# brandonckelly/carma_pack

Measured on AMD Instinct MI355X. Metric: Kalman log-lik evals/sec, CARMA(5,3) n=270, higher is better.
Workload: dtype f64

## Files before the change

### carma_pack_amd/csrc/carma_pipew.h

```cpp
#pragma once
#include <hip/hip_runtime.h>

#include "carma_core.h"
#include "grp_device.h"
#include "carma_pipe3l.h"
#include "carma_win_asm.h"

namespace carma {

#if defined(CARMA_STAMPS)
#define PIPEW_MARK(i) do { if (mk) { __builtin_amdgcn_sched_barrier(0); mk[i] = clock64(); __builtin_amdgcn_sched_barrier(0); } } while (0)
#else
#define PIPEW_MARK(i) do { } while (0)
#endif

template <int P>
struct PipeWGeom {
    static constexpr int ND = 16 - P;
    static constexpr int NB = 2;
    static constexpr int ENT = P + 1;
    static constexpr int RING_OFF = 0;
    static constexpr int ROT_OFF = NB * ENT * 64;
    static constexpr int HDR_OFF = ROT_OFF + NB * P * 4;
    static constexpr int CONST_OFF = HDR_OFF + NB;
    static constexpr int OUT_OFF = CONST_OFF + 64;
    static constexpr int TAB_OFF = OUT_OFF + 4;
    static constexpr int MRG_OFF = TAB_OFF + MATH_TAB_N / 2;
    static constexpr int MRG_STRIDE = P + 1 + ((P + 1) & 1);
    static constexpr int MRG_X = 0;
    static constexpr int MRG_COL = MRG_X + P * MRG_STRIDE;
    static constexpr int MRG_L = MRG_COL + MRG_STRIDE;
    static constexpr int MRG_T = MRG_L + P * MRG_STRIDE;
    static constexpr int MRG_DOUBLES = MRG_T + P * MRG_STRIDE;
    static constexpr int TH_OFF = MRG_OFF + (2 * MRG_DOUBLES + 1) / 2;
    static constexpr int SCH_OFF = TH_OFF + 128;
    static constexpr int ENTRIES = SCH_OFF + NB * 4 * 2;
    static constexpr int SER_OFF = ENTRIES;
    static __host__ __device__ size_t bytes_with_series(int n) { return BYTES + (size_t)(n + (n & 1)) * 24; }
    static constexpr int NPROD = 3;
    static constexpr size_t BYTES = (size_t)ENTRIES * sizeof(double2);
    static constexpr double LIM_RE = Pipe3LGeom<P>::LIM_RE, LIM_IM = Pipe3LGeom<P>::LIM_IM;
};

CARMA_DEV double exp_step_tab_exact(double a, double dt, const double* tab)
{
    const double x = a * dt;
    const double n1 = rint(x * INV_LN2_32);
    double r = fma3(-n1, LN2_32_HI, x);
    r = fma3(-n1, LN2_32_LO, r);
    r += fma3(a, dt, -x);
    const int i1 = (int)fmin(fmax(n1, -70400.0), 70400.0);
    const double e0 = tab[i1 & 31];
    double pe = 1.0 / 720.0;
    pe = fma3(pe, r, 1.0 / 120.0);
    pe = fma3(pe, r, 1.0 / 24.0);
    pe = fma3(pe, r, 1.0 / 6.0);
    pe = fma3(pe, r, 0.5);
    pe = fma3(pe, r, 1.0);
    return ldexp(fma3(e0, pe * r, e0), i1 >> 5);
}

template <int P, bool TS = false, bool SLDS = false, bool HANDOVER = false, bool FOLD = false, class Tail>
__device__ __forceinline__ void pipew_produce(const Grp<16>& g, int pw, const double* __restrict__ theta,
                                              const double4* __restrict__ series, int n_all, double2* __restrict__ ring, Tail&& tail,
                                              long long* mk = nullptr, const double* __restrict__ lds_t = nullptr,
                                              const double2* __restrict__ lds_yz = nullptr)
{
    using Geo = PipeWGeom<P>;
    constexpr int ND = Geo::ND, NB = Geo::NB, ENT = Geo::ENT;
    if (CARMA_PRIO_P != 0) __builtin_amdgcn_s_setprio(CARMA_PRIO_P);
    static_assert(!FOLD || ((P & 1) && P >= 3 && TS && SLDS && HANDOVER), "the folded form: odd orders of the two-sided kernel with the hand-over");
    constexpr int NPAIR = FOLD ? P / 2 : (P + 1) / 2, PPL = 16 / NPAIR;
    constexpr int NPROD = FOLD ? 2 : Geo::NPROD;
    constexpr int PWD = TS ? 2 : 0;
    constexpr int PWH = FOLD ? 2 : 0;
    constexpr int NIT = (ND + 1 + NPROD * PPL - 1) / (NPROD * PPL);
    const double* tab = reinterpret_cast<const double*>(ring + Geo::TAB_OFF);
    const int lane = g.lane64, l = lane & 15, rowb = lane & ~15, q = lane >> 4;
    const int sub = l / NPAIR, jr = 2 * (l - sub * NPAIR);
    const bool worker = sub < PPL, two = FOLD ? true : jr + 1 < P;
    const bool fold = FOLD && jr == P - 3;
    const bool bwd = TS && (q & 1);
    const int nfwd = (n_all + 1) / 2;
    const int n = TS ? (bwd ? n_all - nfwd : nfwd) : n_all;
    auto recat = [=](int j) {
        const int jj = j < n ? j : n - 1;
        double4 r = series[bwd ? n_all - 1 - jj : jj];
        if (bwd) r.w = -r.w;
        return r;
    };
    int jw = 0;
    double4 rw0, rw1, rw2, rw3;
    if constexpr (!SLDS) {
        rw0 = recat(l);
        rw1 = recat(16 + l);
        rw2 = recat(32 + l);
        rw3 = recat(48 + l);
    }
    auto sidx = [=](int j) {
        const int jj = j < n ? j : n - 1;
        return bwd ? n_all - 1 - jj : jj;
    };
    const double tsgn = bwd ? -1.0 : 1.0;
    double t_first = 0.0, t_meet = 0.0;
    if constexpr (!SLDS) {
        t_first = recat(0).w;
        t_meet = TS ? (bwd ? -series[nfwd - 1].w : series[nfwd - 1].w) : 0.0;
    }
    Cx w = own_ar_root<P>(theta, jr);
    Cx w1 = two ? own_ar_root<P>(theta, jr + 1) : w;
    if (bwd) {
        w.im = -w.im;
        w1.im = -w1.im;
    }
    Cx ws = {0.0, 0.0};
    if constexpr (FOLD) {
        ws = own_ar_root<P>(theta, P - 1);
        if (bwd) ws.im = -ws.im;
    }
    int esig = 0;
    {
        const double sg = fabs(theta[0]);
        (void)frexp(sg, &esig);
        if (!(sg > 0.0 && sg < 1.0 / 0.0)) esig = 0;
    }
    const double mu = theta[2], scale = theta[1];
    const bool realpair = two && w.im == 0.0;
    if (pw == PWH && l >= ND) {
#pragma unroll
        for (int b = 0; b < NB; b++) {
#pragma unroll
            for (int r = 0; r < P; r++) ring[Geo::RING_OFF + (b * ENT + r) * 64 + lane] = make_double2(r == l - ND ? 1.0 : 0.0, 0.0);
            ring[Geo::RING_OFF + (b * ENT + P) * 64 + lane] = make_double2(1.0, 0.0);
        }
    }
    double wl = fmax(fmax(fabs(w.re), fabs(w1.re)) * (1.0 / Geo::LIM_RE), fabs(w.im) * (1.0 / Geo::LIM_IM));
    wl = (wl < 1e12) ? wl : ((wl == wl && wl < 1.0 / 0.0) ? 1e12 : 0.0);
    if constexpr (FOLD) {
        double wls = fmax(fabs(ws.re) * (1.0 / Geo::LIM_RE), fabs(ws.im) * (1.0 / Geo::LIM_IM));
        wls = (wls < 1e12) ? wls : ((wls == wls && wls < 1.0 / 0.0) ? 1e12 : 0.0);
        wl = fmax(wl, wls);
    }
    wl = Grp<16>::max(wl);
    int wex;
    (void)frexp(wl, &wex);
    const double sc = wl > 0.0 ? ldexp(1.0, wex) : 0.0;
    const double halfw = sc > 0.0 ? 0.5 / sc : 0.0;
    const double rg0 = exp_neg(w.re * halfw), g0 = recip(rg0);
    double rg1 = rg0, g1 = g0;
    if (realpair) {
        rg1 = exp_neg(w1.re * halfw);
        g1 = recip(rg1);
    }
    double gS = 1.0;
    if constexpr (FOLD) gS = recip(exp_neg(ws.re * halfw));
    int j0 = 0;
    double base = t_first;
    constexpr bool SSCHED = TS && SLDS && HANDOVER;
    int len = 0, jc = 0;
    bool rot = false, last = false, fin = false;
    double dt_rot = 0.0, dta_keep = 0.0;
    double2 dslot = make_double2(1.0, 0.0);
    unsigned long long rbits = 0ull;
    double ecv[NIT], esv[NIT], e1v[NIT];
    double exv[NIT];
    auto sched = [&](bool finflag) __attribute__((always_inline)) {
        jc = j0;
        const int jl = j0 + l;
        double4 rec;
        if constexpr (SLDS) {
            const int si = sidx(jl);
            rec.x = rec.y = rec.z = 0.0;
            rec.w = tsgn * lds_t[si];
            if (pw == PWD) {
                const double2 yz = lds_yz[si];
                rec.y = yz.x;
                rec.z = yz.y;
            }
        } else {
            const int pos = jl - jw, src = rowb + (pos & 15);
            const bool hi = pos >= 16;
            const double w0 = __shfl(rw0.w, src, 64), w1_ = __shfl(rw1.w, src, 64);
            rec.x = rec.y = rec.z = 0.0;
            rec.w = hi ? w1_ : w0;
            if (pw == PWD) {
                const double y0 = __shfl(rw0.y, src, 64), y1 = __shfl(rw1.y, src, 64);
                const double z0 = __shfl(rw0.z, src, 64), z1 = __shfl(rw1.z, src, 64);
                rec.y = hi ? y1 : y0;
                rec.z = hi ? z1 : z0;
            }
        }
        const double tj = rec.w;
        const int left = n - j0;
        const int ncand = left < ND ? (left > 0 ? left : 0) : ND;
        const double t0 = finflag ? t_meet : Grp<16>::template bcast_c<0>(tj);
        const double t_lastc = SLDS ? tsgn * lds_t[sidx(j0 + (ncand > 0 ? ncand - 1 : 0))] : __shfl(tj, rowb + (ncand > 0 ? ncand - 1 : 0), 64);
        const double W = sc > 0.0 ? 1.0 / sc : 1.0 / 0.0;
        rot = finflag || (ncand > 0 && (t_lastc - base) > W);
        dt_rot = t0 - base;
        base = rot ? t0 : base;
        const double dta_l = tj - base;
        dta_keep = dta_l;
        const unsigned long long flb = __ballot(dta_l > W && l < ncand);
        const unsigned cut = (unsigned)(flb >> (16 * q)) & 0xffffu;
        len = cut ? __builtin_ctz(cut) : ncand;
        const bool row_done = j0 + len >= n;
        last = __ballot(!row_done) == 0ull;
        if (pw == PWD) dslot = l < len ? make_double2(rec.z * scale, rec.y - mu) : make_double2(1.0, 0.0);
        j0 += len;
        if (!SLDS && j0 - jw >= 16) {
            rw0 = rw1;
            rw1 = rw2;
            rw2 = rw3;
            jw += 16;
            rw3 = recat(jw + 48 + l);
        }
    };
    double2* schb = ring + Geo::SCH_OFF;
    auto sched_put = [&](int b) __attribute__((always_inline)) {
        if (l == 0) {
            const int bits = jc | (len << 16) | (rot ? 1 << 24 : 0) | (last ? 1 << 25 : 0);
            schb[(b * 4 + q) * 2] = make_double2(__hiloint2double(0, bits), base);
            schb[(b * 4 + q) * 2 + 1] = make_double2(dt_rot, 0.0);
        }
    };
    auto sched_get = [&](int b) __attribute__((always_inline)) {
        const double2 s0 = schb[(b * 4 + q) * 2], s1 = schb[(b * 4 + q) * 2 + 1];
        const int bits = __double2loint(s0.x);
        jc = bits & 0xffff;
        len = (bits >> 16) & 0xff;
        rot = ((bits >> 24) & 1) != 0;
        last = ((bits >> 25) & 1) != 0;
        base = s0.y;
        dt_rot = s1.x;
    };
    auto exps = [&]() __attribute__((always_inline)) {
        if (pw == PWH) rbits = __ballot(rot);
        if constexpr (FOLD) {
            if (pw >= NPROD) return;
        }
#pragma unroll
        for (int it = 0; it < NIT; it++) {
            const int slot = it * NPROD * PPL + pw * PPL + sub;
            const bool is_rot = slot == ND;
            double dts;
            if constexpr (SLDS) {
                dts = tsgn * lds_t[sidx(jc + (slot < ND ? slot : 0))] - base;
            } else {
                dts = __shfl(dta_keep, rowb + (slot < ND ? slot : 0), 64);
            }
            const double dt = is_rot ? dt_rot : dts;
            const bool live = worker && (is_rot ? rot : slot < len);
            double ec = 1.0, es = 0.0, e1 = 1.0;
            if (live) cexp_step_tab<true>(w.re, w.im, dt, &ec, &es, tab);
            e1 = ec;
            if (realpair && live) e1 = exp_neg_tab(w1.re * dt, tab);
            ecv[it] = ec;
            esv[it] = es;
            e1v[it] = e1;
            if constexpr (FOLD) exv[it] = (fold && live) ? exp_step_tab_exact(ws.re, dt, tab) : 1.0;
        }
    };
    PIPEW_MARK(1);
    __syncthreads();
    PIPEW_MARK(2);
    if constexpr (SLDS) {
        base = tsgn * lds_t[sidx(0)];
        t_meet = tsgn * lds_t[nfwd - 1];
    }
    double2 hc_own, hc_par, hc_s = make_double2(0.0, 0.0);
    {
        const double2* cst = ring + Geo::CONST_OFF + rowb;
        if constexpr (FOLD) {
            hc_s = cst[P - 1];
            const double ms = fabs(hc_s.x);
            int es_;
            (void)frexp(ms, &es_);
            if (!(ms > 0.0 && ms < 1.0 / 0.0)) es_ = 0;
            hc_s = make_double2(ldexp(hc_s.x, esig - es_), ldexp(hc_s.y, es_ - esig));
            if (bwd) hc_s = make_double2(hc_s.y, hc_s.x);
        }
        hc_own = cst[jr];
        hc_par = cst[jr + 1 < 16 ? jr + 1 : 15];
        const double m0 = fmax(fabs(hc_own.x), realpair ? 0.0 : fabs(hc_par.x)), m1 = realpair ? fabs(hc_par.x) : m0;
        int e0, e1x;
        (void)frexp(m0, &e0);
        (void)frexp(m1, &e1x);
        if (!(m0 > 0.0 && m0 < 1.0 / 0.0)) e0 = 0;
        if (!(m1 > 0.0 && m1 < 1.0 / 0.0)) e1x = 0;
        hc_own = make_double2(ldexp(hc_own.x, esig - e0), ldexp(hc_own.y, e0 - esig));
        hc_par = make_double2(ldexp(hc_par.x, esig - e1x), ldexp(hc_par.y, e1x - esig));
        if (bwd) {
            hc_own = make_double2(hc_own.y, hc_own.x);
            hc_par = make_double2(hc_par.y, hc_par.x);
        }
    }
#if defined(CARMA_WIN_STAMPS)
    unsigned long long ps_work = 0, ps_wait = 0, ps_t0 = 0, ps_t1 = 0;
    int ps_n = 0;
#define WIN_STAMP(v) asm volatile("s_memtime %0\n\ts_waitcnt lgkmcnt(0)" : "=s"(v)::"memory")
#endif
    for (int c = 0;; c++) {
        const int b = c % NB;
#if defined(CARMA_WIN_STAMPS)
        WIN_STAMP(ps_t0);
#endif
        if (!SSCHED || c == 0)
            sched(fin);
        else if (pw != PWD)
            sched_get(b);
        exps();
        if (pw == PWH && lane == 0)
            reinterpret_cast<unsigned long long*>(ring + Geo::HDR_OFF)[b] =
                ((rbits & 1ull) | ((rbits >> 15) & 2ull) | ((rbits >> 30) & 4ull) | ((rbits >> 45) & 8ull)) | ((TS ? fin : last) ? 256ull : 0ull);
        if (pw == PWD && l < ND) ring[Geo::RING_OFF + (b * ENT + P) * 64 + lane] = dslot;
        if (!FOLD || pw < NPROD) {
#pragma unroll
        for (int it = 0; it < NIT; it++) {
            const int slot = it * NPROD * PPL + pw * PPL + sub;
            const bool is_rot = slot == ND;
            const bool live = worker && (is_rot ? rot : slot < len);
            const double ec = ecv[it], es = esv[it], e1 = e1v[it];
            if (worker && slot < ND) {
                const double gc = ec * g0, gs = es * g0;
                const double inv = recip(fma(gc, gc, gs * gs));
                const double ht = fma(gc, hc_own.x, gs * hc_par.x);
                const double ct = fma(gc, hc_own.y, gs * hc_par.y) * inv;
                double2* dst = ring + Geo::RING_OFF + (b * ENT + jr) * 64 + rowb + slot;
                dst[0] = live ? make_double2(ht, ct) : make_double2(0.0, 0.0);
                if (two) {
                    const double gc1 = e1 * g1, gs1 = es * g1;
                    const double inv1 = realpair ? recip(gc1 * gc1) : inv;
                    const double hp = fma(gc1, hc_par.x, -gs1 * hc_own.x);
                    const double cp = fma(gc1, hc_par.y, -gs1 * hc_own.y) * inv1;
                    dst[64] = live ? make_double2(hp, cp) : make_double2(0.0, 0.0);
                }
                if constexpr (FOLD) {
                    if (fold) {
                        const double ex = exv[it], ez = ex * 0.0;
                        const double gcs = ex * gS, gss = ez * gS;
                        const double invs = recip(fma(gcs, gcs, gss * gss));
                        const double hts = fma(gcs, hc_s.x, gss * 0.0);
                        const double cts = fma(gcs, hc_s.y, gss * 0.0) * invs;
                        dst[128] = live ? make_double2(hts, cts) : make_double2(0.0, 0.0);
                    }
                }
            }
            if (worker && is_rot) {
                double2* dst = ring + Geo::ROT_OFF + (b * P + jr) * 4 + q;
                const double f0 = fin ? g0 : 1.0, f1 = fin ? g1 : 1.0;
                dst[0] = make_double2(ec * f0, es * f0);
                if (two) dst[4] = make_double2(e1 * f1, -es * f1);
                if constexpr (FOLD) {
                    if (fold) {
                        const double ex = exv[it], ez = ex * 0.0;
                        const double fS = fin ? gS : 1.0;
                        dst[8] = make_double2(ex * fS, ez * fS);
                    }
                }
            }
        }
        }
#if defined(CARMA_WIN_STAMPS)
        WIN_STAMP(ps_t1);
        ps_work += ps_t1 - ps_t0;
#endif
        const bool last_c = last, fin_c = fin;
        if (SSCHED && pw == PWD && !(TS ? fin_c : last_c)) {
            sched(last_c);
            sched_put((c + 1) % NB);
        }
        if (c < 3) PIPEW_MARK(3 + 2 * c - (c == 2));
        __syncthreads();
        if (c == 0) PIPEW_MARK(4);
#if defined(CARMA_WIN_STAMPS)
        WIN_STAMP(ps_t0);
        ps_wait += ps_t0 - ps_t1;
        ps_n++;
#endif
        if (TS ? fin_c : last_c) break;
        fin = last_c;
    }
#if defined(CARMA_WIN_STAMPS)
    if (blockIdx.x == 0 && lane == 0)
        printf("window pipeline, producer %d: %d chunks, per chunk %llu cycles of work, %llu at the barrier\n", pw, ps_n,
               ps_work / (unsigned long long)ps_n, ps_wait / (unsigned long long)ps_n);
#endif
    tail(pw);
    if (!TS) __syncthreads();
}

CARMA_DEV double rsqrt_pos(double d)
{
#ifdef __HIPCC__
    const double y0 = __builtin_amdgcn_rsq(d);
    const double e = fma(-d * y0, y0, 1.0);
    return fma(y0, fma(0.375 * e, e, 0.5 * e), y0);
#else
    return 1.0 / sqrt(d);
#endif
}
CARMA_DEV void merge_lds_sync()
{
#ifdef __HIPCC__
    __builtin_amdgcn_fence(__ATOMIC_RELEASE, "wavefront");
    __builtin_amdgcn_wave_barrier();
    __builtin_amdgcn_fence(__ATOMIC_ACQUIRE, "wavefront");
#endif
}
template <int P>
__device__ __forceinline__ void pipew_merge(int lane, const double (&kf)[P], double nu, double2* __restrict__ ring, LogLikAcc& acc,
                                            long long* mk = nullptr)
{
    using Geo = PipeWGeom<P>;
    constexpr int ND = Geo::ND, ST = Geo::MRG_STRIDE;
    const int l = lane & 15, q = lane >> 4;
    const bool bwd = (q & 1) != 0, virt = l >= ND;
    const int j = virt ? l - ND : 0;
    double* mrg = reinterpret_cast<double*>(ring + Geo::MRG_OFF) + (q >> 1) * Geo::MRG_DOUBLES;
    if (!bwd && virt) {
        double* dst = mrg + Geo::MRG_X + j * ST;
#pragma unroll
        for (int r = 0; r < P; r++) dst[r] = kf[r];
        dst[P] = nu;
    }
    merge_lds_sync();
    double S[P], av[P];
#pragma unroll
    for (int i = 0; i < P; i++) {
        S[i] = -mrg[Geo::MRG_X + (i >= j ? j * ST + i : i * ST + j)];
        av[i] = mrg[Geo::MRG_X + i * ST + P];
    }
    double aj = mrg[Geo::MRG_X + j * ST + P];
    int sj = 0;
    double dg = -mrg[Geo::MRG_X + j * ST + j];
    {
        int ex;
        (void)frexp(dg, &ex);
        if (dg > 0.0 && dg < 1.0 / 0.0) sj = -(ex >> 1);
    }
    dg = ldexp(dg, 2 * sj);
    double kfs[P];
    static_for<0, P>([&](auto ic) __attribute__((always_inline)) {
        constexpr int i = decltype(ic)::value;
        const int si = Grp<16>::template bcast_c<ND + i>(sj);
        S[i] = ldexp(S[i], si + sj);
        kfs[i] = ldexp(kf[i], -si - sj);
        av[i] = ldexp(av[i], si);
    });
    aj = ldexp(aj, sj);
    nu = ldexp(nu, -sj);
    PIPEW_MARK(8);
    double Lr[P];
#pragma unroll
    for (int i = 0; i < P; i++) Lr[i] = 0.0;
    bool done = !virt;
    bool exhausted = false;
    static_for<0, P>([&](auto mc) __attribute__((always_inline)) {
        constexpr int m = decltype(mc)::value;
        if (exhausted) return;
        const bool cand = !done && dg > 4e-15;
        unsigned key = cand ? (((unsigned)__double2hiint(dg) & ~0xFu) | (unsigned)(15 - l)) : 0u;
        const double r_own = cand ? rsqrt_pos(dg) : 0.0;
#ifdef __HIPCC__
        key = max(key, (unsigned)__builtin_amdgcn_update_dpp(0, (int)key, DPP_QUAD_XOR1, 0xf, 0xf, true));
        key = max(key, (unsigned)__builtin_amdgcn_update_dpp(0, (int)key, DPP_QUAD_XOR2, 0xf, 0xf, true));
        key = max(key, (unsigned)__builtin_amdgcn_update_dpp(0, (int)key, DPP_ROW_HALF_MIRROR, 0xf, 0xf, true));
        key = max(key, (unsigned)__builtin_amdgcn_update_dpp(0, (int)key, DPP_ROW_MIRROR, 0xf, 0xf, true));
#endif
        const bool any = key != 0u;
        if (__builtin_amdgcn_ballot_w64(any) == 0ull) {
            exhausted = true;
            return;
        }
        const int pl = 15 - (int)(key & 15u);
        const bool isp = any && l == pl;
        const int src = (lane & ~15) + pl;
        double cb[P];
#pragma unroll
        for (int i = 0; i < P; i++) cb[i] = __shfl(S[i] * r_own, src, 64);
        const double r_piv = __shfl(r_own, src, 64);
        const int pc = pl - ND;
        double sp = 0.0;
#pragma unroll
        for (int i = 0; i < P; i++) sp = pc == i ? S[i] : sp;
        const double lj = (any && !done) ? sp * r_piv : 0.0;
        Lr[m] = lj;
#pragma unroll
        for (int i = 0; i < P; i++) S[i] = fma(-cb[i], lj, S[i]);
        dg = fma(-lj, lj, dg);
        done = done || isp;
    });
    PIPEW_MARK(9);
    double T[P];
#pragma unroll
    for (int m = 0; m < P; m++) T[m] = 0.0;
    static_for<0, P>([&](auto kc) __attribute__((always_inline)) {
        constexpr int k = decltype(kc)::value;
#pragma unroll
        for (int m = 0; m < P; m++) T[m] = fma(kfs[k], Grp<16>::template bcast_c<ND + k>(Lr[m]), T[m]);
    });
    double dba = 0.0;
#pragma unroll
    for (int k = 0; k < P; k++) dba = fma(kfs[k], av[k], dba);
    const double uj = -nu - dba;
    PIPEW_MARK(10);
    if (bwd && virt) {
        double* lb = mrg + Geo::MRG_L + j * ST;
        double* tb = mrg + Geo::MRG_T + j * ST;
#pragma unroll
        for (int m = 0; m < P; m++) {
            lb[m] = Lr[m];
            tb[m] = T[m];
        }
        tb[P] = uj;
    }
    merge_lds_sync();
    double Wc[P + 1];
    {
        double tm[P], lm[P], v = 0.0;
#pragma unroll
        for (int i = 0; i < P; i++) {
            tm[i] = mrg[Geo::MRG_T + i * ST + j];
            lm[i] = mrg[Geo::MRG_L + i * ST + j];
            v = fma(lm[i], mrg[Geo::MRG_T + i * ST + P], v);
        }
#pragma unroll
        for (int k = 0; k < P; k++) {
            double w = j == k ? 1.0 : 0.0;
#pragma unroll
            for (int i = 0; i < P; i++) w = fma(mrg[Geo::MRG_L + i * ST + k], tm[i], w);
            Wc[k] = w;
        }
        Wc[P] = v;
    }
    PIPEW_MARK(11);
    double piv = 1.0, s2 = 0.0;
    static_for<0, P>([&](auto kc) __attribute__((always_inline)) {
        constexpr int k = decltype(kc)::value;
        const double dk = Grp<16>::template bcast_c<ND + k>(Wc[k]);
        const double rk = recip(dk);
        if (l == ND + k) {
            piv = Wc[k];
            s2 = Wc[P] * Wc[P] * rk;
        }
        const double f = l > ND + k ? Wc[k] * rk : 0.0;
#pragma unroll
        for (int i = k + 1; i < P + 1; i++) Wc[i] = fma(-Grp<16>::template bcast_c<ND + k>(Wc[i]), f, Wc[i]);
    });
#if defined(CARMA_MERGE_DEBUG)
    if (blockIdx.x == 0 && q < 2 && virt) {
        printf("merge %s lane %d: in kf %.17g %.17g %.17g nu %.17g | sj %d Lr %.6g %.6g %.6g | T %.6g %.6g %.6g | W %.6g %.6g %.6g border %.6g | piv %.17g s2 %.6g dba %.6g aj %.6g\n",
               bwd ? "bwd" : "fwd", j, kf[0], kf[1], kf[P - 1], nu, sj, Lr[0], Lr[1], Lr[P - 1], T[0], T[1], T[P - 1], Wc[0], Wc[1], Wc[P - 1], Wc[P], piv, s2, dba, aj);
    }
#endif
    if (bwd && virt) {
        acc.add_var(piv);
        acc.chi2 += s2 - 2.0 * aj * fma(0.5, dba, nu);
    }
}

template <int P, bool TS = false>
__device__ __forceinline__ double pipew_recur(const Grp<16>& g, const RowConsts<P>& rc, double2* __restrict__ ring, long long* mk = nullptr)
{
    using Geo = PipeWGeom<P>;
    using WA = WinAsm<P>;
    constexpr int ND = Geo::ND, NB = Geo::NB, ENT = Geo::ENT;
    const int lane = g.lane64, l = lane & 15, q = lane >> 4;
    __builtin_amdgcn_s_setprio(CARMA_PRIO_A);
    const bool act = l < P;
    ring[Geo::CONST_OFF + lane] = make_double2(act ? rc.h_own : 0.0, act ? rc.c_own : 0.0);
    __syncthreads();
    double ka[P], ha[P], kb[P], hb[P];
#pragma unroll
    for (int r = 0; r < P; r++) ka[r] = ha[r] = kb[r] = hb[r] = 0.0;
    double mA = 1.0, mB = 1.0, nuA = 0.0, nuB = 0.0;
    LogLikAcc acc;
    acc.init();
    const bool data = l < ND, evn = (l & 1) == 0;
    double2 en[ENT];
    unsigned long long hdr = 0;
    auto load = [&](int b, double2(&e)[ENT], unsigned long long& h) __attribute__((always_inline)) {
#pragma unroll
        for (int r = 0; r < ENT; r++) e[r] = ring[Geo::RING_OFF + (b * ENT + r) * 64 + lane];
        h = reinterpret_cast<const unsigned long long*>(ring + Geo::HDR_OFF)[b];
    };
    auto start = [&](int b, const double(&kold)[P], double(&kn)[P], double(&hn)[P]) __attribute__((always_inline)) {
        const double nuF = (ND & 1) ? nuB : nuA;
        double nun = en[P].y, mn = en[P].x;
        double cn[P];
#pragma unroll
        for (int r = 0; r < P; r++) {
            hn[r] = en[r].x;
            cn[r] = en[r].y;
        }
        if (__builtin_expect((hdr & 0xfull) != 0ull, 0)) {
            double cr[P], sr[P], hx[P];
            const bool mine = ((hdr >> q) & 1ull) != 0ull;
#pragma unroll
            for (int r = 0; r < P; r++) {
                const double2 v = ring[Geo::ROT_OFF + (b * P + r) * 4 + q];
                cr[r] = v.x;
                sr[r] = (r ^ 1) < P ? v.y : 0.0;
            }
#pragma unroll
            for (int r = 0; r < P; r++) {
                const int rp = (r ^ 1) < P ? (r ^ 1) : r;
                hx[r] = fma(cr[r], hn[r], sr[r] * hn[rp]);
                kn[r] = mine ? 0.0 : cn[r];
            }
            WA::init(kn, nun, kold, nuF, hx);
            double t[P];
#pragma unroll
            for (int r = 0; r < P; r++) t[r] = kn[r];
#pragma unroll
            for (int r = 0; r < P; r++) {
                const int rp = (r ^ 1) < P ? (r ^ 1) : r;
                kn[r] = fma(cr[r], t[r], -(sr[r] * t[rp])) + (mine ? cn[r] : 0.0);
            }
        } else {
#pragma unroll
            for (int r = 0; r < P; r++) kn[r] = cn[r];
            WA::init(kn, nun, kold, nuF, hn);
        }
#pragma unroll
        for (int r = 0; r < P; r++) mn = fma(hn[r], kn[r], mn);
        mA = mB = mn;
        nuA = nuB = nun;
    };
    auto chunk = [&](double(&kk)[P], double(&hh)[P], double(&kn)[P], double(&hn)[P], int c) __attribute__((always_inline)) -> bool {
        const bool last = !TS && (hdr & 256ull) != 0ull;
        double2 en2[ENT];
        unsigned long long hdr2 = 0;
        if (c > 0) {
            __syncthreads();
            if (!last) load((c + 1) % NB, en2, hdr2);
        }
        __builtin_amdgcn_sched_barrier(0);
        WA::chunk(kk, hh, mA, mB, nuA, nuB);
        __builtin_amdgcn_sched_barrier(0);
        if (c == 0) {
            __syncthreads();
            if (!last) load((c + 1) % NB, en2, hdr2);
        }
        {
            const double varF = data ? (evn ? mA : mB) : 1.0, innF = data ? (evn ? nuA : nuB) : 0.0;
            acc.add_var(varF);
            acc.chi2 += innF * (recip(varF) * innF);
        }
        if (last) return true;
#pragma unroll
        for (int r = 0; r < ENT; r++) en[r] = en2[r];
        hdr = hdr2;
        start((c + 1) % NB, kk, kn, hn);
        return TS && (hdr & 256ull) != 0ull;
    };
    __syncthreads();
    PIPEW_MARK(3);
    load(0, en, hdr);
    start(0, ka, kb, hb);
    PIPEW_MARK(4);
    bool fin_in_a = true;
    for (int c = 0;; c += 2) {
        if (chunk(kb, hb, ka, ha, c)) break;
        if (chunk(ka, ha, kb, hb, c + 1)) {
            fin_in_a = false;
            break;
        }
    }
    PIPEW_MARK(5);
    if constexpr (TS) {
        double kf[P];
#pragma unroll
        for (int r = 0; r < P; r++) kf[r] = fin_in_a ? ka[r] : kb[r];
        pipew_merge<P>(lane, kf, nuA, ring, acc, mk);
    }
    PIPEW_MARK(6);
    double ll = Grp<16>::sum(acc.total());
    if constexpr (TS) ll += __shfl_xor(ll, 16, 64);
    return ll;
}

}
```

Measured before the change: 49.88 million.

## Restructure merge pivoted Cholesky to overlap rsqrt and fold T build into steps

Splits the rsqrt into a seed and a refinement so the seed for the next pivot step is issued before the rank-one update, overlapping its latency. Pivot rows are now fetched by register broadcast and a binary select tree instead of P shuffles per step. The T accumulation and the LDS stores of L and T move inside each elimination step, with non-owning lanes writing to a dead scratch area so the stores need no branch. The later W build reads L and u from register broadcasts instead of LDS. This adds code complexity and some redundant writes to scratch LDS.

```diff
diff --git a/carma_pack_amd/csrc/carma_pipew.h b/carma_pack_amd/csrc/carma_pipew.h
--- a/carma_pack_amd/csrc/carma_pipew.h
+++ b/carma_pack_amd/csrc/carma_pipew.h
@@ -10,8 +10,10 @@
 
 #if defined(CARMA_STAMPS)
 #define PIPEW_MARK(i) do { if (mk) { __builtin_amdgcn_sched_barrier(0); mk[i] = clock64(); __builtin_amdgcn_sched_barrier(0); } } while (0)
+#define PIPEW_COUNT(i, n) do { if (mk) mk[i] = mk[0] + (n); } while (0)
 #else
 #define PIPEW_MARK(i) do { } while (0)
+#define PIPEW_COUNT(i, n) do { } while (0)
 #endif
 
 template <int P>
@@ -390,16 +392,24 @@
     if (!TS) __syncthreads();
 }
 
-CARMA_DEV double rsqrt_pos(double d)
+CARMA_DEV double rsqrt_seed(double d)
 {
 #ifdef __HIPCC__
-    const double y0 = __builtin_amdgcn_rsq(d);
+    return __builtin_amdgcn_rsq(d);
+#else
+    return 1.0 / sqrt(d);
+#endif
+}
+CARMA_DEV double rsqrt_finish(double d, double y0)
+{
+#ifdef __HIPCC__
     const double e = fma(-d * y0, y0, 1.0);
     return fma(y0, fma(0.375 * e, e, 0.5 * e), y0);
 #else
-    return 1.0 / sqrt(d);
-#endif
-}
+    return y0;
+#endif
+}
+CARMA_DEV double rsqrt_pos(double d) { return rsqrt_finish(d, rsqrt_seed(d)); }
 CARMA_DEV void merge_lds_sync()
 {
 #ifdef __HIPCC__
@@ -407,6 +417,23 @@
     __builtin_amdgcn_wave_barrier();
     __builtin_amdgcn_fence(__ATOMIC_ACQUIRE, "wavefront");
 #endif
+}
+template <int P>
+CARMA_DEV double merge_pick(const double (&v)[P], int idx)
+{
+    double t[P];
+#pragma unroll
+    for (int i = 0; i < P; i++) t[i] = v[i];
+#pragma unroll
+    for (int s = 1; s < P; s <<= 1) {
+        const bool up = (idx & s) != 0;
+#pragma unroll
+        for (int i = 0; i + s < P; i += 2 * s) {
+            const double lo = t[i], hi = t[i + s];
+            t[i] = up ? hi : lo;
+        }
+    }
+    return t[0];
 }
 template <int P>
 __device__ __forceinline__ void pipew_merge(int lane, const double (&kf)[P], double nu, double2* __restrict__ ring, LogLikAcc& acc,
@@ -451,87 +478,105 @@
     aj = ldexp(aj, sj);
     nu = ldexp(nu, -sj);
     PIPEW_MARK(8);
-    double Lr[P];
+    double Lr[P], tz = 0.0;
+#pragma unroll
+    for (int k = 0; k < P; k++) tz = fma(kfs[k], 0.0, tz);
 #pragma unroll
     for (int i = 0; i < P; i++) Lr[i] = 0.0;
+    double dba = 0.0;
+#pragma unroll
+    for (int k = 0; k < P; k++) dba = fma(kfs[k], av[k], dba);
+    const double uj = -nu - dba;
+    constexpr int NJUNK = (P + 1) * ST - (P - 1);
+    static_assert(Geo::MRG_X == 0 && Geo::MRG_COL == P * ST && Geo::MRG_L == (P + 1) * ST && NJUNK >= 1, "the dead area in front of L");
+    const bool keeps = bwd && virt;
+    double* const lb = keeps ? mrg + Geo::MRG_L + j * ST : mrg + Geo::MRG_X + (lane & 31) % NJUNK;
+    double* const tb = keeps ? mrg + Geo::MRG_T + j * ST : lb;
     bool done = !virt;
     bool exhausted = false;
-    static_for<0, P>([&](auto mc) __attribute__((always_inline)) {
-        constexpr int m = decltype(mc)::value;
-        if (exhausted) return;
+    [[maybe_unused]] int nsteps = 0;
+    unsigned key = 0u;
+    double r_own = 0.0;
+    auto offer = [&](double y0) __attribute__((always_inline)) {
         const bool cand = !done && dg > 4e-15;
-        unsigned key = cand ? (((unsigned)__double2hiint(dg) & ~0xFu) | (unsigned)(15 - l)) : 0u;
-        const double r_own = cand ? rsqrt_pos(dg) : 0.0;
+        key = cand ? (((unsigned)__double2hiint(dg) & ~0xFu) | (unsigned)(15 - l)) : 0u;
 #ifdef __HIPCC__
         key = max(key, (unsigned)__builtin_amdgcn_update_dpp(0, (int)key, DPP_QUAD_XOR1, 0xf, 0xf, true));
         key = max(key, (unsigned)__builtin_amdgcn_update_dpp(0, (int)key, DPP_QUAD_XOR2, 0xf, 0xf, true));
         key = max(key, (unsigned)__builtin_amdgcn_update_dpp(0, (int)key, DPP_ROW_HALF_MIRROR, 0xf, 0xf, true));
         key = max(key, (unsigned)__builtin_amdgcn_update_dpp(0, (int)key, DPP_ROW_MIRROR, 0xf, 0xf, true));
 #endif
+        const double r_all = rsqrt_finish(dg, y0);
+        r_own = cand ? r_all : 0.0;
+    };
+    offer(rsqrt_seed(dg));
+    static_for<0, P>([&](auto mc) __attribute__((always_inline)) {
+        constexpr int m = decltype(mc)::value;
+        if (exhausted) return;
         const bool any = key != 0u;
         if (__builtin_amdgcn_ballot_w64(any) == 0ull) {
             exhausted = true;
+            if (keeps) {
+#pragma unroll
+                for (int r = m; r < P; r++) {
+                    lb[r] = 0.0;
+                    tb[r] = tz;
+                }
+            }
             return;
         }
+        nsteps++;
         const int pl = 15 - (int)(key & 15u);
         const bool isp = any && l == pl;
-        const int src = (lane & ~15) + pl;
-        double cb[P];
-#pragma unroll
-        for (int i = 0; i < P; i++) cb[i] = __shfl(S[i] * r_own, src, 64);
-        const double r_piv = __shfl(r_own, src, 64);
         const int pc = pl - ND;
-        double sp = 0.0;
-#pragma unroll
-        for (int i = 0; i < P; i++) sp = pc == i ? S[i] : sp;
-        const double lj = (any && !done) ? sp * r_piv : 0.0;
+        const double lraw = merge_pick<P>(S, pc) * __shfl(r_own, (lane & ~15) + pl, 64);
+        const bool live = any & !done;
+        const double lj = live ? lraw : 0.0;
         Lr[m] = lj;
-#pragma unroll
-        for (int i = 0; i < P; i++) S[i] = fma(-cb[i], lj, S[i]);
         dg = fma(-lj, lj, dg);
         done = done || isp;
+        [[maybe_unused]] double y0 = 0.0;
+        if constexpr (m + 1 < P) y0 = rsqrt_seed(dg);
+        double lc[P], tm = 0.0;
+        static_for<0, P>([&](auto ic) __attribute__((always_inline)) {
+            constexpr int i = decltype(ic)::value;
+            lc[i] = Grp<16>::template bcast_c<ND + i>(lj);
+            double sn = fma(-lc[i], lj, S[i]);
+            if constexpr (m + 1 < P) asm volatile("" : "+v"(sn));
+            S[i] = sn;
+        });
+        if constexpr (m + 1 < P) offer(y0);
+#pragma unroll
+        for (int k = 0; k < P; k++) tm = fma(kfs[k], lc[k], tm);
+        lb[m] = lj;
+        tb[m] = tm;
     });
+    PIPEW_COUNT(12, nsteps);
     PIPEW_MARK(9);
-    double T[P];
-#pragma unroll
-    for (int m = 0; m < P; m++) T[m] = 0.0;
-    static_for<0, P>([&](auto kc) __attribute__((always_inline)) {
-        constexpr int k = decltype(kc)::value;
-#pragma unroll
-        for (int m = 0; m < P; m++) T[m] = fma(kfs[k], Grp<16>::template bcast_c<ND + k>(Lr[m]), T[m]);
-    });
-    double dba = 0.0;
-#pragma unroll
-    for (int k = 0; k < P; k++) dba = fma(kfs[k], av[k], dba);
-    const double uj = -nu - dba;
     PIPEW_MARK(10);
-    if (bwd && virt) {
-        double* lb = mrg + Geo::MRG_L + j * ST;
-        double* tb = mrg + Geo::MRG_T + j * ST;
-#pragma unroll
-        for (int m = 0; m < P; m++) {
-            lb[m] = Lr[m];
-            tb[m] = T[m];
-        }
-        tb[P] = uj;
-    }
     merge_lds_sync();
     double Wc[P + 1];
     {
-        double tm[P], lm[P], v = 0.0;
+        double tm[P], lm[P];
 #pragma unroll
         for (int i = 0; i < P; i++) {
             tm[i] = mrg[Geo::MRG_T + i * ST + j];
             lm[i] = mrg[Geo::MRG_L + i * ST + j];
-            v = fma(lm[i], mrg[Geo::MRG_T + i * ST + P], v);
-        }
-#pragma unroll
-        for (int k = 0; k < P; k++) {
+        }
+        static_for<0, P>([&](auto kc) __attribute__((always_inline)) {
+            constexpr int k = decltype(kc)::value;
             double w = j == k ? 1.0 : 0.0;
-#pragma unroll
-            for (int i = 0; i < P; i++) w = fma(mrg[Geo::MRG_L + i * ST + k], tm[i], w);
+            static_for<0, P>([&](auto ic) __attribute__((always_inline)) {
+                constexpr int i = decltype(ic)::value;
+                w = fma(Grp<16>::template bcast_c<ND + i>(Lr[k]), tm[i], w);
+            });
             Wc[k] = w;
-        }
+        });
+        double v = 0.0;
+        static_for<0, P>([&](auto ic) __attribute__((always_inline)) {
+            constexpr int i = decltype(ic)::value;
+            v = fma(lm[i], Grp<16>::template bcast_c<ND + i>(uj), v);
+        });
         Wc[P] = v;
     }
     PIPEW_MARK(11);
```

Result: no change. 50.17 million, median of 6 (+0.6%).
